# ignacio-rocco/detectorch

Hardware: AMD Instinct MI355X
Metric: images/sec Mask R-CNN R-50-FPN 1333x800 (region-proposal hot path) (higher is better)
Workload: dtype f32

## Files before the change

### detectorch_amd/csrc/roi_align_common.h

```cpp
#pragma once
#include "dtc_common.h"

namespace dtc {

struct RoiAlignParams {
  dtc_feat_level lv[DTC_MAX_LEVELS];
  const float* rois;
  const int32_t* roi_levels;
  const int32_t* roi_order;
  const float* roi_desc;
  void* out;
  int n_levels, channels, roi_cols, n_rois, pooled_h, pooled_w, sampling_ratio, ch_tile;
  int ch_block;
  int cts64;
  int xcd_remap;
  const void* prep = nullptr;
};

constexpr int kXcds = 8;
__device__ __forceinline__ int xcd_work_item(int b, int n, int enabled) {
  if (!enabled || n < 2 * kXcds) return b;
  const int x = b % kXcds, j = b / kXcds;
  const int q = n / kXcds, r = n - q * kXcds;
  return x * q + min(x, r) + j;
// ... 18 lines not shown
  e.l = valid ? l : 0.f;
  e.h = valid ? h : 0.f;
  return e;
}

struct RoiHead {
  int r, lvl, b;
  float sw, sh, rw, rh;
  float bin_h, bin_w;
  int gh, gw;
  float count, inv_count;
};

struct RoiRaw { float4 d0, d1; };

__device__ __forceinline__ RoiRaw load_roi_raw(const RoiAlignParams& p, int ri) {
  RoiRaw w;
  if (p.roi_desc) {
    w.d0 = reinterpret_cast<const float4*>(p.roi_desc)[(size_t)ri * 2];
    w.d1 = reinterpret_cast<const float4*>(p.roi_desc)[(size_t)ri * 2 + 1];
  } else {
    const int r = p.roi_order ? p.roi_order[ri] : ri;
    const int lvl = p.roi_levels ? p.roi_levels[r] : 0;
    const float* roi = p.rois + (size_t)r * p.roi_cols;
    float b = 0.f;
    if (p.roi_cols == 5) { b = roi[0]; roi++; }
    w.d0 = make_float4(b, roi[0], roi[1], roi[2]);
    w.d1 = make_float4(roi[3], (float)lvl, (float)r, 0.f);
  }
  return w;
}

__device__ __forceinline__ RoiHead roi_head_from_raw(const RoiAlignParams& p, const RoiRaw& w) {
  RoiHead h;
  h.b = (int)w.d0.x; h.lvl = (int)w.d1.y; h.r = (int)w.d1.z;
  const float x1 = w.d0.y, y1 = w.d0.z, x2 = w.d0.w, y2 = w.d1.x;
  h.sw = h.sh = 0.f; h.rw = h.rh = 1.f; h.bin_h = h.bin_w = 1.f; h.gh = h.gw = 1; h.count = 1.f; h.inv_count = 1.f;
  if (h.lvl < 0 || h.lvl >= p.n_levels) return h;
  const float s = p.lv[h.lvl].spatial_scale;
  h.sw = x1 * s; h.sh = y1 * s;
  const float ew = x2 * s, eh = y2 * s;
  h.rw = fmaxf(ew - h.sw, 1.f); h.rh = fmaxf(eh - h.sh, 1.f);
  h.bin_h = fdiv(h.rh, (float)p.pooled_h); h.bin_w = fdiv(h.rw, (float)p.pooled_w);
  h.gh = p.sampling_ratio > 0 ? p.sampling_ratio : (int)ceilf(fdiv(h.rh, (float)p.pooled_h));
  h.gw = p.sampling_ratio > 0 ? p.sampling_ratio : (int)ceilf(fdiv(h.rw, (float)p.pooled_w));
  const int gg = h.gh * h.gw;
  h.count = (float)gg;
  h.inv_count = ((gg & (gg - 1)) == 0) ? fdiv(1.f, h.count) : 0.f;
  return h;
}

__device__ __forceinline__ RoiHead load_roi_head(const RoiAlignParams& p, int ri) {
  return roi_head_from_raw(p, load_roi_raw(p, ri));
}

typedef float f32x2 __attribute__((ext_vector_type(2)));
template <typename T> __device__ __forceinline__ f32x2 mul_pair16(uint32_t u, float w);
template <> __device__ __forceinline__ f32x2 mul_pair16<__half>(uint32_t u, float w) {
  f32x2 r;
  asm("v_fma_mix_f32 %0, %2, %3, %4 op_sel:[0,0,0] op_sel_hi:[1,0,0]\n\tv_fma_mix_f32 %1, %2, %3, %4 op_sel:[1,0,0] op_sel_hi:[1,0,0]"
      : "=&v"(r.x), "=&v"(r.y) : "v"(u), "v"(w), "s"(-0.0f));
  return r;
}
template <> __device__ __forceinline__ f32x2 mul_pair16<bf16_t>(uint32_t u, float w) {
  const f32x2 v = {__uint_as_float(u << 16), __uint_as_float(u & 0xffff0000u)};
  return v * w;
}
template <> __device__ __forceinline__ f32x2 mul_pair16<float>(uint32_t, float) { return f32x2{0.f, 0.f}; }

template <typename T> __device__ __forceinline__ void fma_pair16(f32x2& acc, uint32_t u, float w);
template <> __device__ __forceinline__ void fma_pair16<__half>(f32x2& acc, uint32_t u, float w) {
  asm("v_fma_mix_f32 %0, %2, %3, %0 op_sel:[0,0,0] op_sel_hi:[1,0,0]\n\tv_fma_mix_f32 %1, %2, %3, %1 op_sel:[1,0,0] op_sel_hi:[1,0,0]"
      : "+v"(acc.x), "+v"(acc.y) : "v"(u), "v"(w));
}
template <> __device__ __forceinline__ void fma_pair16<bf16_t>(f32x2& acc, uint32_t u, float w) {
  const f32x2 v = {__uint_as_float(u << 16), __uint_as_float(u & 0xffff0000u)};
  const f32x2 w2 = {w, w};
  acc = __builtin_elementwise_fma(v, w2, acc);
}
template <> __device__ __forceinline__ void fma_pair16<float>(f32x2&, uint32_t, float) {}

bool roi_align_tile_supported(const RoiAlignParams& p, int in_dtype, int out_dtype);
int launch_roi_align_tile(const RoiAlignParams& p, int in_dtype, int out_dtype, hipStream_t stream);
bool roi_align_map_supported(const RoiAlignParams& p, int in_dtype, int out_dtype);
int launch_roi_align_map(const RoiAlignParams& p, int in_dtype, int out_dtype, hipStream_t stream);
void roi_align_set_exact(int exact);
int roi_align_get_exact();
size_t roi_align_map_workspace_bytes(int n_rois);
int launch_roi_align_map_ws(const RoiAlignParams& p, int in_dtype, int out_dtype, void* workspace, size_t workspace_bytes, hipStream_t stream);

bool roi_align_nhwc_lds_supported(const RoiAlignParams& p, int in_dtype, int out_dtype);
int launch_roi_align_nhwc_lds(const RoiAlignParams& p, int in_dtype, int out_dtype, hipStream_t stream);

bool roi_align_nhwc16_supported(const RoiAlignParams& p, int in_dtype, int out_dtype);
int launch_roi_align_nhwc16(const RoiAlignParams& p, int in_dtype, int out_dtype, hipStream_t stream);

}
```

### detectorch_amd/csrc/roi_align_tile.hip

```cpp
#include <stdlib.h>

#include <mutex>
#include <type_traits>

#include "roi_align_common.h"

namespace dtc {

constexpr int kTileMaxK = 32;
constexpr int kTileRoiBytes = 48, kTileGroupBytes = 32;
constexpr int kTileHdrBytes = kTileMaxK * (kTileRoiBytes + kTileGroupBytes) + 16;
template <int NT> struct TileShape;
template <> struct TileShape<256> { static constexpr int kUnits = 8, kWaves = 3, kLdsKB = 52, kWaves16 = 4, kLds16KB = 38; };

struct TileRoi {
  int lvl, b, x0, x1, y0, y1, r, valid;
  float sh, sw, bin_h, bin_w;
};
static_assert(sizeof(TileRoi) == kTileRoiBytes, "TileRoi layout");
struct TileGroup { int first, count, kind, x0, x1, y0, y1, pad; };
enum { kGrpPool = 0, kGrpZero = 1, kGrpAbsent = 2, kGrpGather = 3 };

typedef uint32_t u32x4 __attribute__((ext_vector_type(4)));
typedef uint32_t u32x2 __attribute__((ext_vector_type(2)));
typedef float f32x2 __attribute__((ext_vector_type(2)));
typedef float f32x4 __attribute__((ext_vector_type(4)));
__device__ __forceinline__ __amdgpu_buffer_rsrc_t make_srd(const void* base) {
  return __builtin_amdgcn_make_buffer_rsrc(const_cast<void*>(base), 0, 0xffffffff, 0x00020000);
}
template <typename TIn> struct Piece4;
template <> struct Piece4<float> {
  typedef float4 Raw;
  static __device__ __forceinline__ Raw raw(__amdgpu_buffer_rsrc_t r, uint32_t voff, uint32_t soff) { return ld(r, voff, soff); }
  static __device__ __forceinline__ float4 ld(__amdgpu_buffer_rsrc_t r, uint32_t voff, uint32_t soff) {
    const u32x4 v = __builtin_amdgcn_raw_buffer_load_b128(r, voff, soff, 0);
    return make_float4(__uint_as_float(v.x), __uint_as_float(v.y), __uint_as_float(v.z), __uint_as_float(v.w));
  }
};
template <> struct Piece4<__half> {
  typedef u32x2 Raw;
  static __device__ __forceinline__ Raw raw(__amdgpu_buffer_rsrc_t r, uint32_t voff, uint32_t soff) { return __builtin_amdgcn_raw_buffer_load_b64(r, voff, soff, 0); }
  static __device__ __forceinline__ float4 ld(__amdgpu_buffer_rsrc_t r, uint32_t voff, uint32_t soff) {
    const u32x2 v = __builtin_amdgcn_raw_buffer_load_b64(r, voff, soff, 0);
    const uint32_t x = v.x, y = v.y;
    const __half2 a = *reinterpret_cast<const __half2*>(&x), b = *reinterpret_cast<const __half2*>(&y);
    return make_float4(__low2float(a), __high2float(a), __low2float(b), __high2float(b));
  }
};
template <> struct Piece4<bf16_t> {
  typedef u32x2 Raw;
  static __device__ __forceinline__ Raw raw(__amdgpu_buffer_rsrc_t r, uint32_t voff, uint32_t soff) { return __builtin_amdgcn_raw_buffer_load_b64(r, voff, soff, 0); }
  static __device__ __forceinline__ float4 ld(__amdgpu_buffer_rsrc_t r, uint32_t voff, uint32_t soff) {
    const u32x2 v = __builtin_amdgcn_raw_buffer_load_b64(r, voff, soff, 0);
    return bf16x4_to_f32(make_uint2(v.x, v.y));
  }
};

__device__ __forceinline__ int uni(int v) { return __builtin_amdgcn_readfirstlane(v); }

#ifdef DTC_TILE_TRACE
constexpr int kTraceSlots = 16;
__device__ unsigned long long g_tile_trace[kTraceSlots * 16384];
struct TileTrace {
  unsigned long long last, acc[kTraceSlots];
  __device__ __forceinline__ void start() { for (int i = 0; i < kTraceSlots; i++) acc[i] = 0; last = __builtin_readcyclecounter(); }
  __device__ __forceinline__ void mark(int i) { const unsigned long long n = __builtin_readcyclecounter(); acc[i] += n - last; last = n; }
};
#define TT_MARK(i) tt.mark(i)
#else
struct TileTrace {};
#define TT_MARK(i) ((void)0)
#endif

template <typename TIn> struct TileLds { typedef float T; static constexpr int kSlot = 16, kShift = 4; };
template <> struct TileLds<__half> { typedef uint16_t T; static constexpr int kSlot = 8, kShift = 3; };
template <> struct TileLds<bf16_t> { typedef uint16_t T; static constexpr int kSlot = 8, kShift = 3; };

template <typename TIn, int NT> struct TileBounds { static constexpr int kWaves = TileShape<NT>::kWaves; };
template <int NT> struct TileBounds<__half, NT> { static constexpr int kWaves = TileShape<NT>::kWaves16; };
template <int NT> struct TileBounds<bf16_t, NT> { static constexpr int kWaves = TileShape<NT>::kWaves16; };

__device__ __forceinline__ int tile_phys(int px) { return px + (px >> 3); }

struct TileItem {
  int a[2][2][4];
  float yl[2], yh[2], xl[2], xh[2];
  bool on;
};

template <typename TOut> __device__ __forceinline__ void store_quad(TOut* d, float4 v);
template <> __device__ __forceinline__ void store_quad<float>(float* d, float4 v) { store_stream16(d, v); }
template <> __device__ __forceinline__ void store_quad<__half>(__half* d, float4 v) {
  const __half2 a = __floats2half2_rn(v.x, v.y), b = __floats2half2_rn(v.z, v.w);
  store_stream8(d, *reinterpret_cast<const uint32_t*>(&a), *reinterpret_cast<const uint32_t*>(&b));
}
template <> __device__ __forceinline__ void store_quad<bf16_t>(bf16_t* d, float4 v) {
  store_stream8(d, (uint32_t)from_f32<bf16_t>(v.x).bits | ((uint32_t)from_f32<bf16_t>(v.y).bits << 16),
                (uint32_t)from_f32<bf16_t>(v.z).bits | ((uint32_t)from_f32<bf16_t>(v.w).bits << 16));
}

enum { kStageScalar = 0, kStageVec = 1, kStageVecUnaligned = 2 };

struct TileGeom {
  int first, count;
  int y0, x0a, ngx, npos;
  int plane;
  int nq_pass;
  int mode;
};

template <typename TIn, typename TOut, int NT, bool FUSED>
__device__ __forceinline__ void tile_passes(const RoiAlignParams& p, const dtc_feat_level& L, const TIn* fbase, int c0, int nc,
                                            int bins, float* slab, typename TileLds<TIn>::T* win, const TileRoi* troi, const TileGeom& g,
                                            const TileItem& it, int rl, int bin, TileTrace& tt) {
  constexpr int NW = NT / 64;
  constexpr int U = TileShape<NT>::kUnits;
  typedef typename TileLds<TIn>::T TL;
  constexpr bool L16 = sizeof(TL) == 2;
  constexpr int SB = TileLds<TIn>::kSlot;
  const int tid = threadIdx.x, lane = tid & 63, wv = tid >> 6, pl = lane & 15, cl = (lane >> 4) & 3;
  const int npos = g.npos, ngx = g.ngx, plane = g.plane, nq_pass = g.nq_pass;
  const int nchunk = (npos + 15) >> 4;
  const int KC = ceil_div(nchunk, NW);
  const float rinv = 1.0f / (float)ngx;
  const int nq_tot = ceil_div(nc, 4);
  const bool vec = g.mode != kStageScalar;
  uint32_t uoff[U];
  int ulds[U];
  const int nu = KC * nq_pass;
  if (vec) {
    const int sh32 = (int)L.stride_h, sc32 = (int)L.stride_c;
    int q = 0, i = 0;
#pragma unroll
    for (int u = 0; u < U; u++) {
      const bool dup = u >= nu;
      const int pos = min((wv + (dup ? 0 : i) * NW) * 16 + pl, npos - 1);
      const int row = (int)(((float)pos + 0.5f) * rinv);
      const int gx = pos - row * ngx;
      const int qq = dup ? 0 : q;
      int col = g.x0a + 4 * gx, sft = 0;
      if (g.mode == kStageVecUnaligned) { sft = max(0, col + 3 - (L.width - 1)); col -= sft; }
      uoff[u] = ((uint32_t)((g.y0 + row) * sh32 + col + (4 * qq + cl) * sc32) * (uint32_t)sizeof(TIn)) | ((uint32_t)sft << 30);
      ulds[u] = qq * plane * 4 + ((4 * pos + (pos >> 1)) << 2) + cl;
      if (++i == KC) { i = 0; q++; }
    }
  }
  const __amdgpu_buffer_rsrc_t srd = make_srd(fbase);
  const uint32_t pass_bytes = (uint32_t)(L.stride_c * (int64_t)sizeof(TIn));
  typename Piece4<TIn>::Raw v[U];
  auto issue = [&](int cs) {
    const uint32_t soff = (uint32_t)cs * pass_bytes;
    if (g.mode == kStageVec) {
#pragma unroll
      for (int u = 0; u < U; u++) v[u] = Piece4<TIn>::raw(srd, uoff[u], soff);
    } else {
#pragma unroll
      for (int u = 0; u < U; u++) v[u] = Piece4<TIn>::raw(srd, uoff[u] & 0x3fffffffu, soff);
    }
  };
  auto commit_as = [&](auto shifted_tag) {
    constexpr bool SHIFTED = decltype(shifted_tag)::value;
    if constexpr (SHIFTED) asm volatile("" ::: "memory");
#pragma unroll
    for (int u = 0; u < U; u++) {
      if constexpr (L16) {
        uint32_t w0 = v[u].x & 0xffffu, w1 = v[u].x >> 16, w2 = v[u].y & 0xffffu, w3 = v[u].y >> 16;
        if constexpr (SHIFTED) {
          const uint32_t sft = uoff[u] >> 30;
          w0 = sft == 0 ? w0 : sft == 1 ? w1 : sft == 2 ? w2 : w3;
          w1 = sft == 0 ? w1 : sft == 1 ? w2 : w3;
          w2 = sft == 0 ? w2 : w3;
        }
        TL* d = win + ulds[u];
        d[0] = (TL)w0; d[4] = (TL)w1; d[8] = (TL)w2; d[12] = (TL)w3;
      } else {
        float4 w = v[u];
        if constexpr (SHIFTED) {
          const uint32_t sft = uoff[u] >> 30;
          w.x = sft == 0 ? w.x : sft == 1 ? w.y : sft == 2 ? w.z : w.w;
          w.y = sft == 0 ? w.y : sft == 1 ? w.z : w.w;
          w.z = sft == 0 ? w.z : w.w;
        }
        TL* d = win + ulds[u];
        d[0] = w.x; d[4] = w.y; d[8] = w.z; d[12] = w.w;
// ... 122 lines not shown
    TT_MARK(4);
    if (nq_prev) store_slab(cs_prev, nq_prev);
    TT_MARK(5);
    __syncthreads();
    TT_MARK(6);
    if (vec && qs + nq_pass < nq_tot) issue(cs + 4 * nq_pass);
    TT_MARK(7);
    if (it.on) {
      float* so = slab + rl * (4 * nq_cur * bins) + bin;
#pragma unroll 1
      for (int q = 0; q < nq_cur; q++) {
        const char* wq = reinterpret_cast<const char*>(win) + uni(q * plane * SB);
        f32x2 a01 = {0.f, 0.f}, a23 = {0.f, 0.f};
#pragma unroll
        for (int iy = 0; iy < 2; iy++) {
          if constexpr (L16 && FUSED) {
            u32x2 t[2][4];
#pragma unroll
            for (int ix = 0; ix < 2; ix++)
#pragma unroll
              for (int k = 0; k < 4; k++)
                t[ix][k] = *reinterpret_cast<const u32x2*>(__builtin_assume_aligned(wq + it.a[iy][ix][k], 8));
#pragma unroll
            for (int ix = 0; ix < 2; ix++) {
              const float w1 = it.yh[iy] * it.xh[ix], w2 = it.yh[iy] * it.xl[ix];
              const float w3 = it.yl[iy] * it.xh[ix], w4 = it.yl[iy] * it.xl[ix];
              fma_pair16<TIn>(a01, t[ix][0].x, w1); fma_pair16<TIn>(a23, t[ix][0].y, w1);
              fma_pair16<TIn>(a01, t[ix][1].x, w2); fma_pair16<TIn>(a23, t[ix][1].y, w2);
              fma_pair16<TIn>(a01, t[ix][2].x, w3); fma_pair16<TIn>(a23, t[ix][2].y, w3);
              fma_pair16<TIn>(a01, t[ix][3].x, w4); fma_pair16<TIn>(a23, t[ix][3].y, w4);
            }
          } else if constexpr (L16) {
            u32x2 t[2][4];
#pragma unroll
            for (int ix = 0; ix < 2; ix++)
#pragma unroll
              for (int k = 0; k < 4; k++)
                t[ix][k] = *reinterpret_cast<const u32x2*>(__builtin_assume_aligned(wq + it.a[iy][ix][k], 8));
#pragma unroll
            for (int ix = 0; ix < 2; ix++) {
              const float w1 = it.yh[iy] * it.xh[ix], w2 = it.yh[iy] * it.xl[ix];
              const float w3 = it.yl[iy] * it.xh[ix], w4 = it.yl[iy] * it.xl[ix];
              f32x2 s01 = mul_pair16<TIn>(t[ix][0].x, w1) + mul_pair16<TIn>(t[ix][1].x, w2);
              s01 = s01 + mul_pair16<TIn>(t[ix][2].x, w3);
              s01 = s01 + mul_pair16<TIn>(t[ix][3].x, w4);
              f32x2 s23 = mul_pair16<TIn>(t[ix][0].y, w1) + mul_pair16<TIn>(t[ix][1].y, w2);
              s23 = s23 + mul_pair16<TIn>(t[ix][2].y, w3);
              s23 = s23 + mul_pair16<TIn>(t[ix][3].y, w4);
              a01 = a01 + s01; a23 = a23 + s23;
            }
          } else {
            f32x4 t[2][4];
#pragma unroll
            for (int ix = 0; ix < 2; ix++)
#pragma unroll
              for (int k = 0; k < 4; k++)
                t[ix][k] = *reinterpret_cast<const f32x4*>(__builtin_assume_aligned(wq + it.a[iy][ix][k], 16));
#pragma unroll
            for (int ix = 0; ix < 2; ix++) {
              const float w1 = it.yh[iy] * it.xh[ix], w2 = it.yh[iy] * it.xl[ix];
              const float w3 = it.yl[iy] * it.xh[ix], w4 = it.yl[iy] * it.xl[ix];
              a01 += w1 * t[ix][0].lo + w2 * t[ix][1].lo + w3 * t[ix][2].lo + w4 * t[ix][3].lo;
              a23 += w1 * t[ix][0].hi + w2 * t[ix][1].hi + w3 * t[ix][2].hi + w4 * t[ix][3].hi;
            }
          }
          __builtin_amdgcn_sched_barrier(0);
        }
        float* o = so + uni(4 * q * bins);
        const float a0 = a01.x, a1 = a01.y, a2 = a23.x, a3 = a23.y;
        o[0] = a0 * 0.25f; o[bins] = a1 * 0.25f; o[2 * bins] = a2 * 0.25f; o[3 * bins] = a3 * 0.25f;
      }
    }
    TT_MARK(8);
    __syncthreads();
    TT_MARK(9);
    cs_prev = cs; nq_prev = nq_cur;
  }
  if (nq_prev) store_slab(cs_prev, nq_prev);
  TT_MARK(10);
}
#endif


__device__ __forceinline__ int tile_work_item(int b, int n, int reverse) {
  if (n < 2 * kXcds || (reverse & 2)) return (reverse & 1) ? n - 1 - b : b;
  const int x = b % kXcds, j = b / kXcds;
  const int q = n / kXcds, r = n - q * kXcds;
  const int start = x * q + min(x, r), qx = q + (x < r ? 1 : 0);
  return start + ((reverse & 1) ? qx - 1 - j : j);
}

template <typename TIn, typename TOut, int NT, bool FUSED>
__global__ __launch_bounds__(NT, (TileBounds<TIn, NT>::kWaves)) void roi_align_fwd_tile(RoiAlignParams p, int kgroup, int lds_bytes, int nq_cap, int merge_pct, int reverse) {
  extern __shared__ __attribute__((aligned(16))) unsigned char smem[];
  TileRoi* troi = reinterpret_cast<TileRoi*>(smem);
  TileGroup* tgrp = reinterpret_cast<TileGroup*>(smem + kTileMaxK * kTileRoiBytes);
  int* ngp = reinterpret_cast<int*>(smem + kTileMaxK * (kTileRoiBytes + kTileGroupBytes));
  const int slab_bytes = kgroup * p.pooled_h * p.pooled_w * 16 * nq_cap;
  float* slab = reinterpret_cast<float*>(smem + kTileHdrBytes);
  typedef typename TileLds<TIn>::T TL;
  constexpr int SB = TileLds<TIn>::kSlot;
  TL* win = reinterpret_cast<TL*>(smem + kTileHdrBytes + slab_bytes);
  const int win_bytes = lds_bytes - kTileHdrBytes - slab_bytes;
  constexpr int NW = NT / 64;
  constexpr int kMaxPos = TileShape<NT>::kUnits * NW * 16;
  const int tid = threadIdx.x;
  const int nct = ceil_div(p.channels, p.ch_block);
  int wi = tile_work_item(blockIdx.x, gridDim.x, reverse);
  int grp = wi / nct;
  int c0 = (wi - grp * nct) * p.ch_block;
  {
    const int ngrp = (int)gridDim.x / nct;
    if ((reverse & 4) && ngrp % kXcds == 0 && ngrp >= 2 * kXcds) {
      const int x = blockIdx.x % kXcds, j = blockIdx.x / kXcds, ngx = ngrp / kXcds;
      const int cbi = j / ngx, gl = j - cbi * ngx;
      grp = x * ngx + ((reverse & 1) ? ngx - 1 - gl : gl);
      c0 = cbi * p.ch_block;
      wi = grp * nct + cbi;
    }
  }
  const int nc = min(p.ch_block, p.channels - c0);
  const int bins = p.pooled_h * p.pooled_w;
  const int K = kgroup;
  TileTrace tt;
#ifdef DTC_TILE_TRACE
  tt.start();
  const unsigned long long wall0 = __builtin_amdgcn_s_memrealtime();
#endif

  if (tid < 64) {
    TileRoi t;
    t.lvl = -1; t.b = 0; t.x0 = t.x1 = t.y0 = t.y1 = 0; t.r = 0; t.valid = 0; t.sh = t.sw = 0.f; t.bin_h = t.bin_w = 1.f;
    const int ri = grp * K + tid;
    if (tid < K && ri < p.n_rois) {
      const RoiHead hd = load_roi_head(p, ri);
      t.valid = 1; t.r = hd.r; t.b = hd.b; t.sh = hd.sh; t.sw = hd.sw; t.bin_h = hd.bin_h; t.bin_w = hd.bin_w;
      if (hd.lvl >= 0 && hd.lvl < p.n_levels) {
        t.lvl = hd.lvl;
        const int H = p.lv[hd.lvl].height, W = p.lv[hd.lvl].width;
        t.y0 = make_axis(hd.sh, hd.bin_h, 0, 0, 2, H).lo;
        t.y1 = make_axis(hd.sh, hd.bin_h, p.pooled_h - 1, 1, 2, H).hi;
        t.x0 = make_axis(hd.sw, hd.bin_w, 0, 0, 2, W).lo;
        t.x1 = make_axis(hd.sw, hd.bin_w, p.pooled_w - 1, 1, 2, W).hi;
      }
    }
    if (tid < K) {
      troi[tid] = t;
      *reinterpret_cast<uint64_t*>(&troi[tid].x0) = ((uint64_t)(uint32_t)t.r * (uint64_t)p.channels + (uint64_t)c0) * (uint64_t)(p.pooled_h * p.pooled_w);
    }
    auto bc = [](int v, int k) { return __builtin_amdgcn_readlane(v, k); };
    int ng = 0, k = 0;
    while (k < K) {
      const int ks = uni(k);
      const int a_lvl = bc(t.lvl, ks), a_b = bc(t.b, ks), a_valid = bc(t.valid, ks);
      const int a_x0 = bc(t.x0, ks), a_x1 = bc(t.x1, ks), a_y0 = bc(t.y0, ks), a_y1 = bc(t.y1, ks);
      TileGroup g;
      g.first = k; g.count = 1; g.x0 = a_x0; g.x1 = a_x1; g.y0 = a_y0; g.y1 = a_y1; g.pad = 0;
      if (!a_valid) g.kind = kGrpAbsent;
      else if (a_lvl < 0) g.kind = kGrpZero;
      else {
        const int ngx0 = (a_x1 >> 2) - (a_x0 >> 2) + 1, th0 = a_y1 - a_y0 + 1, npos0 = th0 * ngx0;
        if (npos0 > kMaxPos || (4 * npos0 + (npos0 >> 1) + 1) * SB > win_bytes || bins > NT) {
          g.kind = kGrpGather;
        } else {
          g.kind = kGrpPool;
          long long sum_px = (long long)th0 * (a_x1 - a_x0 + 1);
          while (k + g.count < K && (g.count + 1) * bins <= NT) {
            const int js = uni(k + g.count);
            const int n_lvl = bc(t.lvl, js), n_b = bc(t.b, js), n_valid = bc(t.valid, js);
            if (!n_valid || n_lvl != a_lvl || n_b != a_b) break;
            const int n_x0 = bc(t.x0, js), n_x1 = bc(t.x1, js), n_y0 = bc(t.y0, js), n_y1 = bc(t.y1, js);
            const int ux0 = min(g.x0, n_x0), ux1 = max(g.x1, n_x1), uy0 = min(g.y0, n_y0), uy1 = max(g.y1, n_y1);
            const int ungx = (ux1 >> 2) - (ux0 >> 2) + 1, uth = uy1 - uy0 + 1, unpos = uth * ungx;
// ... 104 lines not shown
    unsigned long long* o = g_tile_trace + (size_t)blockIdx.x * kTraceSlots;
    for (int i = 0; i < 11; i++) o[i] = tt.acc[i];
    o[11] = wall0; o[12] = __builtin_amdgcn_s_memrealtime();
    o[13] = (unsigned long long)ngroups; o[14] = (unsigned long long)__builtin_amdgcn_s_getreg((4 << 0) | (0 << 6) | (31 << 11));
    o[15] = (unsigned long long)wi;
  }
#endif
}

#ifdef DTC_TILE_TRACE
}
extern "C" __attribute__((visibility("default"))) int dtc_debug_tile_trace(void* host_dst, size_t bytes) {
  return hipMemcpyFromSymbol(host_dst, HIP_SYMBOL(dtc::g_tile_trace), bytes, 0, hipMemcpyDeviceToHost) == hipSuccess ? 0 : -1;
}
namespace dtc {
#endif

struct TileConfig {
  int nt = 256;
  int lds_kb = 0;
  int lds16_kb = 0;
  int k = 0;
  int ch_block = 0;
  int merge_pct = 250;
  int nq_cap = 0;
  int reverse = 1;
  int cb_major = 1;
};
static const TileConfig& tile_config() {
  static const TileConfig cfg = [] {
    TileConfig c;
    if (const char* e = getenv("DTC_RA_TILE_CBMAJOR")) c.cb_major = atoi(e) != 0;
    if (const char* e = getenv("DTC_RA_TILE_LDS16_KB")) { const int v = atoi(e); if (v >= 36 && v <= 156) c.lds16_kb = v; }
    if (const char* e = getenv("DTC_RA_TILE_CHBLOCK")) { const int v = atoi(e); if (v >= 4 && (v & 3) == 0) c.ch_block = v; }
    return c;
  }();
  return cfg;
}

template <typename TIn, typename TOut, int NT, bool FUSED>
static int launch_tile_nt(RoiAlignParams p, hipStream_t stream) {
  const TileConfig& cfg = tile_config();
  const int bins = p.pooled_h * p.pooled_w;
  int K = cfg.k ? cfg.k : NT / bins;
  K = K < 1 ? 1 : (K > kTileMaxK ? kTileMaxK : K);
  if (K * bins > NT) K = NT / bins;
  if (K < 1) return DTC_EUNSUPPORTED;
  const int lds_b = (sizeof(TIn) == 2 ? (cfg.lds16_kb ? cfg.lds16_kb : TileShape<NT>::kLds16KB) : cfg.lds_kb ? cfg.lds_kb : TileShape<NT>::kLdsKB) * 1024;
  static std::once_flag once;
  static hipError_t attr_rc = hipSuccess;
  std::call_once(once, [] {
    attr_rc = hipFuncSetAttribute(reinterpret_cast<const void*>(roi_align_fwd_tile<TIn, TOut, NT, FUSED>),
                                  hipFuncAttributeMaxDynamicSharedMemorySize, 160 * 1024);
  });
  if (attr_rc != hipSuccess) return DTC_ELAUNCH;
  const int nq_cap = cfg.nq_cap ? cfg.nq_cap : 4;
  if (kTileHdrBytes + K * bins * 16 * nq_cap + 20 * 1024 > lds_b) return DTC_EUNSUPPORTED;
  const int ngrp = ceil_div(p.n_rois, K);
  int cb = cfg.ch_block ? cfg.ch_block : ((long long)ngrp * ceil_div(p.channels, 128) >= 6144 ? 128 : 64);
  while (!cfg.ch_block && cb > 32 && (long long)ngrp * ceil_div(p.channels, cb) < 2048) cb >>= 1;
  p.ch_block = cb;
  const int nct = ceil_div(p.channels, p.ch_block);
  hipLaunchKernelGGL((roi_align_fwd_tile<TIn, TOut, NT, FUSED>), dim3((unsigned)ngrp * nct), dim3(NT), lds_b, stream, p, K, lds_b, nq_cap, cfg.merge_pct, (cfg.reverse ? 1 : 0) | (p.xcd_remap ? 0 : 2) | (cfg.cb_major ? 4 : 0));
  DTC_CHECK_LAUNCH();
  return DTC_OK;
}

template <typename TIn, typename TOut>
static int launch_tile_t(const RoiAlignParams& p, hipStream_t stream) {
  if constexpr (sizeof(TIn) == 2) { if (!roi_align_get_exact()) return launch_tile_nt<TIn, TOut, 256, true>(p, stream); }
  return launch_tile_nt<TIn, TOut, 256, false>(p, stream);
}

bool roi_align_tile_supported(const RoiAlignParams& p, int in_dtype, int out_dtype) {
  if (p.sampling_ratio != 2) return false;
  if (p.pooled_h * p.pooled_w > tile_config().nt) return false;
  const bool f = in_dtype == DTC_F32, h = in_dtype == DTC_F16, b = in_dtype == DTC_BF16;
  return (f && (out_dtype == DTC_F32 || out_dtype == DTC_F16 || out_dtype == DTC_BF16)) ||
         (h && (out_dtype == DTC_F32 || out_dtype == DTC_F16)) || (b && (out_dtype == DTC_F32 || out_dtype == DTC_BF16));
}

int launch_roi_align_tile(const RoiAlignParams& p, int in_dtype, int out_dtype, hipStream_t stream) {
  if (p.n_rois == 0) return DTC_OK;
  if (in_dtype == DTC_F32 && out_dtype == DTC_F32) return launch_tile_t<float, float>(p, stream);
  if (in_dtype == DTC_F16 && out_dtype == DTC_F32) return launch_tile_t<__half, float>(p, stream);
  if (in_dtype == DTC_F16 && out_dtype == DTC_F16) return launch_tile_t<__half, __half>(p, stream);
  if (in_dtype == DTC_F32 && out_dtype == DTC_F16) return launch_tile_t<float, __half>(p, stream);
  if (in_dtype == DTC_BF16 && out_dtype == DTC_F32) return launch_tile_t<bf16_t, float>(p, stream);
  if (in_dtype == DTC_BF16 && out_dtype == DTC_BF16) return launch_tile_t<bf16_t, bf16_t>(p, stream);
  if (in_dtype == DTC_F32 && out_dtype == DTC_BF16) return launch_tile_t<float, bf16_t>(p, stream);
  return DTC_EUNSUPPORTED;
}

}
```

Before: 14370.

## Add dedicated mask-head RoIAlign kernel with per-ROI channel-block tiling

Adds a specialized RoIAlign kernel for large pooled outputs (over 128 bins, e.g. the 14x14 mask head). Each block handles one ROI and one channel block: it stages the ROI's feature window into LDS with buffer loads double-buffered across channel quads, then computes bilinear samples from LDS, with XCD-aware work ordering. The tile launcher dispatches to this path when it is supported. Shared helpers move into a new header. This adds a separate code path whose benefit depends on how many ROIs and which pooled sizes the benchmark actually uses.

```diff
diff --git a/detectorch_amd/csrc/roi_align_common.h b/detectorch_amd/csrc/roi_align_common.h
--- a/detectorch_amd/csrc/roi_align_common.h
+++ b/detectorch_amd/csrc/roi_align_common.h
@@ -124,6 +124,8 @@
 
 bool roi_align_tile_supported(const RoiAlignParams& p, int in_dtype, int out_dtype);
 int launch_roi_align_tile(const RoiAlignParams& p, int in_dtype, int out_dtype, hipStream_t stream);
+bool roi_align_mask_supported(const RoiAlignParams& p, int in_dtype, int out_dtype);
+int launch_roi_align_mask(const RoiAlignParams& p, int in_dtype, int out_dtype, hipStream_t stream);
 bool roi_align_map_supported(const RoiAlignParams& p, int in_dtype, int out_dtype);
 int launch_roi_align_map(const RoiAlignParams& p, int in_dtype, int out_dtype, hipStream_t stream);
 void roi_align_set_exact(int exact);
diff --git a/detectorch_amd/csrc/roi_align_mask.hip b/detectorch_amd/csrc/roi_align_mask.hip
--- /dev/null
+++ b/detectorch_amd/csrc/roi_align_mask.hip
@@ -0,0 +1,330 @@
+#include <stdlib.h>
+
+#include <mutex>
+
+#include "roi_align_stage.h"
+
+namespace dtc {
+
+constexpr int kMaskNT = 256;
+constexpr int kMaskUnits = 8;
+template <typename TIn> struct MaskShape { static constexpr int kWaves = 3, kLdsKB = 52, kQuads = 8; };
+template <> struct MaskShape<__half> { static constexpr int kWaves = 4, kLdsKB = 38, kQuads = 4; };
+template <> struct MaskShape<bf16_t> { static constexpr int kWaves = 4, kLdsKB = 38, kQuads = 4; };
+
+__device__ __forceinline__ void mask_work_item(int b, int n_rows, int nct, int& row, int& cb) {
+  if (n_rows % kXcds == 0 && n_rows >= 2 * kXcds) {
+    const int x = b % kXcds, j = b / kXcds, ngx = n_rows / kXcds;
+    cb = j / ngx;
+    row = x * ngx + (ngx - 1 - (j - cb * ngx));
+  } else {
+    const int wi = tile_work_item(b, n_rows * nct, 1);
+    row = wi / nct;
+    cb = wi - row * nct;
+  }
+}
+
+template <typename TIn, typename TOut>
+__global__ __launch_bounds__(kMaskNT, MaskShape<TIn>::kWaves) void roi_align_fwd_mask(RoiAlignParams p, int lds_bytes, int nq_cap) {
+  extern __shared__ __attribute__((aligned(16))) unsigned char smem[];
+  typedef typename TileLds<TIn>::T TL;
+  constexpr bool L16 = sizeof(TL) == 2;
+  constexpr int SB = TileLds<TIn>::kSlot, SS = TileLds<TIn>::kShift;
+  constexpr int NT = kMaskNT, NW = NT / 64, U = kMaskUnits;
+  const int tid = threadIdx.x, lane = tid & 63, wv = tid >> 6, pl = lane & 15, cl = (lane >> 4) & 3;
+  const int bins = p.pooled_h * p.pooled_w;
+  const int nc = p.ch_block;
+  const int nct = p.channels / nc;
+  int row, cb;
+  mask_work_item(blockIdx.x, p.n_rois, nct, row, cb);
+  const int c0 = cb * nc;
+  const RoiHead hd = load_roi_head(p, row);
+  TOut* out = reinterpret_cast<TOut*>(p.out) + ((size_t)hd.r * p.channels + c0) * bins;
+  if (hd.lvl < 0 || hd.lvl >= p.n_levels) {
+    for (int o = tid; o < nc * bins; o += NT) out[o] = from_f32<TOut>(0.f);
+    return;
+  }
+  const dtc_feat_level L = p.lv[hd.lvl];
+  const TIn* fbase = reinterpret_cast<const TIn*>(L.data) + (int64_t)hd.b * L.stride_n + (int64_t)c0 * L.stride_c;
+  const int y0 = make_axis(hd.sh, hd.bin_h, 0, 0, 2, L.height).lo;
+  const int y1 = make_axis(hd.sh, hd.bin_h, p.pooled_h - 1, 1, 2, L.height).hi;
+  const int x0 = make_axis(hd.sw, hd.bin_w, 0, 0, 2, L.width).lo;
+  const int x1 = make_axis(hd.sw, hd.bin_w, p.pooled_w - 1, 1, 2, L.width).hi;
+  const int x0a = x0 & ~3, ngx = (x1 >> 2) - (x0 >> 2) + 1, tw = 4 * ngx;
+  const int npos = (y1 - y0 + 1) * ngx;
+  const int plane = 4 * npos + (npos >> 1) + 1;
+  const int nchunk = (npos + 15) >> 4, KC = ceil_div(nchunk, NW);
+  const int slab_bytes = bins * 16 * nq_cap;
+  const int img_bytes = lds_bytes - slab_bytes;
+  float* slab = reinterpret_cast<float*>(smem);
+  TL* win = reinterpret_cast<TL*>(smem + slab_bytes);
+
+  if (KC > U || plane * SB > img_bytes) {
+    for (int o = tid; o < nc * bins; o += NT) {
+      const int c = o / bins, bin = o - c * bins;
+      const int ph = bin / p.pooled_w, pw = bin - ph * p.pooled_w;
+      const TIn* d = fbase + (int64_t)c * L.stride_c;
+      float acc = 0.f;
+      for (int iy = 0; iy < 2; iy++) {
+        const AxisEntry y = make_axis(hd.sh, hd.bin_h, ph, iy, 2, L.height);
+        const int64_t ylo = (int64_t)y.lo * L.stride_h, yhi = (int64_t)y.hi * L.stride_h;
+        for (int ix = 0; ix < 2; ix++) {
+          const AxisEntry x = make_axis(hd.sw, hd.bin_w, pw, ix, 2, L.width);
+          const int64_t xlo = (int64_t)x.lo * L.stride_w, xhi = (int64_t)x.hi * L.stride_w;
+          const float w1 = y.h * x.h, w2 = y.h * x.l, w3 = y.l * x.h, w4 = y.l * x.l;
+          acc += w1 * to_f32<TIn>(d[ylo + xlo]) + w2 * to_f32<TIn>(d[ylo + xhi]) + w3 * to_f32<TIn>(d[yhi + xlo]) +
+                 w4 * to_f32<TIn>(d[yhi + xhi]);
+        }
+      }
+      out[o] = from_f32<TOut>(acc * 0.25f);
+    }
+    return;
+  }
+  const bool al16 = ((L.width | L.stride_h | L.stride_c | L.stride_n) & 3) == 0 &&
+                    (reinterpret_cast<uintptr_t>(L.data) & (4 * sizeof(TIn) - 1)) == 0;
+  const int nq_tot = nc >> 2;
+  int nq_pass = max(1, min(min(img_bytes / (plane * SB), U / KC), min(nq_tot, nq_cap)));
+  while (nq_tot % nq_pass) nq_pass--;
+
+  const int nu = KC * nq_pass;
+  const float rinv = 1.0f / (float)ngx;
+  uint32_t uoff[U];
+  int ulds[U];
+  {
+    const int sh32 = (int)L.stride_h, sc32 = (int)L.stride_c;
+    int q = 0, i = 0;
+#pragma unroll
+    for (int u = 0; u < U; u++) {
+      const bool dup = u >= nu;
+      const int pos = min((wv + (dup ? 0 : i) * NW) * 16 + pl, npos - 1);
+      const int r = (int)(((float)pos + 0.5f) * rinv);
+      const int gx = pos - r * ngx;
+      const int qq = dup ? 0 : q;
+      int col = x0a + 4 * gx, sft = 0;
+      if (!al16) { sft = max(0, col + 3 - (L.width - 1)); col -= sft; }
+      uoff[u] = ((uint32_t)((y0 + r) * sh32 + col + (4 * qq + cl) * sc32) * (uint32_t)sizeof(TIn)) | ((uint32_t)sft << 30);
+      ulds[u] = qq * plane * 4 + ((4 * pos + (pos >> 1)) << 2) + cl;
+      if (++i == KC) { i = 0; q++; }
+    }
+  }
+  const __amdgpu_buffer_rsrc_t srd = make_srd(fbase);
+  const uint32_t pass_bytes = (uint32_t)(L.stride_c * (int64_t)sizeof(TIn));
+  typename Piece4<TIn>::Raw v[U];
+  auto issue = [&](int cs) {
+    const uint32_t soff = (uint32_t)cs * pass_bytes;
+    if (al16) {
+#pragma unroll
+      for (int u = 0; u < U; u++) v[u] = Piece4<TIn>::raw(srd, uoff[u], soff);
+    } else {
+#pragma unroll
+      for (int u = 0; u < U; u++) v[u] = Piece4<TIn>::raw(srd, uoff[u] & 0x3fffffffu, soff);
+    }
+  };
+  auto commit_as = [&](auto shifted_tag) {
+    constexpr bool SHIFTED = decltype(shifted_tag)::value;
+    if constexpr (SHIFTED) asm volatile("" ::: "memory");
+#pragma unroll
+    for (int u = 0; u < U; u++) {
+      if constexpr (L16) {
+        uint32_t w0 = v[u].x & 0xffffu, w1 = v[u].x >> 16, w2 = v[u].y & 0xffffu, w3 = v[u].y >> 16;
+        if constexpr (SHIFTED) {
+          const uint32_t sft = uoff[u] >> 30;
+          w0 = sft == 0 ? w0 : sft == 1 ? w1 : sft == 2 ? w2 : w3;
+          w1 = sft == 0 ? w1 : sft == 1 ? w2 : w3;
+          w2 = sft == 0 ? w2 : w3;
+        }
+        TL* d = win + ulds[u];
+        d[0] = (TL)w0; d[4] = (TL)w1; d[8] = (TL)w2; d[12] = (TL)w3;
+      } else {
+        float4 w = v[u];
+        if constexpr (SHIFTED) {
+          const uint32_t sft = uoff[u] >> 30;
+          w.x = sft == 0 ? w.x : sft == 1 ? w.y : sft == 2 ? w.z : w.w;
+          w.y = sft == 0 ? w.y : sft == 1 ? w.z : w.w;
+          w.z = sft == 0 ? w.z : w.w;
+        }
+        TL* d = win + ulds[u];
+        d[0] = w.x; d[4] = w.y; d[8] = w.z; d[12] = w.w;
+      }
+    }
+  };
+  auto commit = [&]() {
+    if (!al16) commit_as(std::true_type{}); else commit_as(std::false_type{});
+  };
+  auto store_slab = [&](int cs, int nq) {
+    const int n4 = nq * bins;
+    TOut* o = out + cs * bins;
+    for (int idx = tid; idx < n4; idx += NT) store_quad<TOut>(o + 4 * idx, reinterpret_cast<const float4*>(slab)[idx]);
+  };
+
+  issue(0);
+
+  const bool on = tid < bins;
+  const int bin = on ? tid : 0;
+  const int ph = bin / p.pooled_w, pw = bin - ph * p.pooled_w;
+  int a[2][2][4];
+  float yl[2], yh[2], xl[2], xh[2];
+  {
+    int ylo[2], yhi[2], xlo[2], xhi[2];
+#pragma unroll
+    for (int i = 0; i < 2; i++) {
+      const AxisEntry ey = make_axis(hd.sh, hd.bin_h, ph, i, 2, L.height);
+      const AxisEntry ex = make_axis(hd.sw, hd.bin_w, pw, i, 2, L.width);
+      yl[i] = ey.l; yh[i] = ey.h; xl[i] = ex.l; xh[i] = ex.h;
+      ylo[i] = (ey.lo - y0) * tw; yhi[i] = (ey.hi - y0) * tw;
+      xlo[i] = ex.lo - x0a; xhi[i] = ex.hi - x0a;
+    }
+#pragma unroll
+    for (int iy = 0; iy < 2; iy++)
+#pragma unroll
+      for (int ix = 0; ix < 2; ix++) {
+        int t0 = tile_phys(ylo[iy] + xlo[ix]) << SS, t1 = tile_phys(ylo[iy] + xhi[ix]) << SS;
+        int t2 = tile_phys(yhi[iy] + xlo[ix]) << SS, t3 = tile_phys(yhi[iy] + xhi[ix]) << SS;
+        asm volatile("" : "+v"(t0), "+v"(t1), "+v"(t2), "+v"(t3));
+        a[iy][ix][0] = t0; a[iy][ix][1] = t1; a[iy][ix][2] = t2; a[iy][ix][3] = t3;
+      }
+  }
+
+  int cs_prev = 0, nq_prev = 0;
+#pragma unroll 1
+  for (int qs = 0; qs < nq_tot; qs += nq_pass) {
+    const int cs = 4 * qs;
+    commit();
+    if (nq_prev) store_slab(cs_prev, nq_prev);
+    __syncthreads();
+    if (qs + nq_pass < nq_tot) issue(cs + 4 * nq_pass);
+    if (on) {
+      float* so = slab + bin;
+#pragma unroll 1
+      for (int q = 0; q < nq_pass; q++) {
+        const char* wq = reinterpret_cast<const char*>(win) + uni(q * plane * SB);
+        f32x2 a01 = {0.f, 0.f}, a23 = {0.f, 0.f};
+#pragma unroll
+        for (int iy = 0; iy < 2; iy++) {
+          if constexpr (L16) {
+            u32x2 t[2][4];
+#pragma unroll
+            for (int ix = 0; ix < 2; ix++)
+#pragma unroll
+              for (int k = 0; k < 4; k++) t[ix][k] = *reinterpret_cast<const u32x2*>(__builtin_assume_aligned(wq + a[iy][ix][k], 8));
+#pragma unroll
+            for (int ix = 0; ix < 2; ix++) {
+              const float w1 = yh[iy] * xh[ix], w2 = yh[iy] * xl[ix];
+              const float w3 = yl[iy] * xh[ix], w4 = yl[iy] * xl[ix];
+              f32x2 s01 = mul_pair16<TIn>(t[ix][0].x, w1) + mul_pair16<TIn>(t[ix][1].x, w2);
+              s01 = s01 + mul_pair16<TIn>(t[ix][2].x, w3);
+              s01 = s01 + mul_pair16<TIn>(t[ix][3].x, w4);
+              f32x2 s23 = mul_pair16<TIn>(t[ix][0].y, w1) + mul_pair16<TIn>(t[ix][1].y, w2);
+              s23 = s23 + mul_pair16<TIn>(t[ix][2].y, w3);
+              s23 = s23 + mul_pair16<TIn>(t[ix][3].y, w4);
+              a01 = a01 + s01; a23 = a23 + s23;
+            }
+          } else {
+            f32x4 t[2][4];
+#pragma unroll
+            for (int ix = 0; ix < 2; ix++)
+#pragma unroll
+              for (int k = 0; k < 4; k++) t[ix][k] = *reinterpret_cast<const f32x4*>(__builtin_assume_aligned(wq + a[iy][ix][k], 16));
+#pragma unroll
+            for (int ix = 0; ix < 2; ix++) {
+              const float w1 = yh[iy] * xh[ix], w2 = yh[iy] * xl[ix];
+              const float w3 = yl[iy] * xh[ix], w4 = yl[iy] * xl[ix];
+              a01 += w1 * t[ix][0].lo + w2 * t[ix][1].lo + w3 * t[ix][2].lo + w4 * t[ix][3].lo;
+              a23 += w1 * t[ix][0].hi + w2 * t[ix][1].hi + w3 * t[ix][2].hi + w4 * t[ix][3].hi;
+            }
+          }
+          __builtin_amdgcn_sched_barrier(0);
+        }
+        float* o = so + uni(4 * q * bins);
+        o[0] = a01.x * 0.25f; o[bins] = a01.y * 0.25f; o[2 * bins] = a23.x * 0.25f; o[3 * bins] = a23.y * 0.25f;
+      }
+    }
+    __syncthreads();
+    cs_prev = cs; nq_prev = nq_pass;
+  }
+  store_slab(cs_prev, nq_prev);
+}
+
+struct MaskConfig {
+  int enabled = 1;
+  int ch_block = 0;
+  int lds_kb = 0;
+  int quads = 0;
+};
+static const MaskConfig& mask_config() {
+  static const MaskConfig cfg = [] {
+    MaskConfig c;
+    if (const char* e = getenv("DTC_RA_MASK")) c.enabled = atoi(e) != 0;
+    if (const char* e = getenv("DTC_RA_MASK_CHBLOCK")) { const int v = atoi(e); if (v == 32 || v == 64 || v == 128) c.ch_block = v; }
+    if (const char* e = getenv("DTC_RA_MASK_LDS_KB")) { const int v = atoi(e); if (v >= 32 && v <= 156) c.lds_kb = v; }
+    if (const char* e = getenv("DTC_RA_MASK_QUADS")) { const int v = atoi(e); if (v >= 1 && v <= 8) c.quads = v; }
+    return c;
+  }();
+  return cfg;
+}
+
+static int mask_ch_block(const RoiAlignParams& p) {
+  const MaskConfig& cfg = mask_config();
+  if (cfg.ch_block) return p.channels % cfg.ch_block == 0 ? cfg.ch_block : 0;
+  int cb = 64;
+  while (cb > 32 && (long long)p.n_rois * (p.channels / cb) < 2048) cb >>= 1;
+  return p.channels % cb == 0 ? cb : (p.channels % 32 == 0 ? 32 : 0);
+}
+
+bool roi_align_mask_supported(const RoiAlignParams& p, int in_dtype, int out_dtype) {
+  const int bins = p.pooled_h * p.pooled_w;
+  if (!mask_config().enabled || !p.roi_desc || p.sampling_ratio != 2 || bins <= 128 || bins > kMaskNT) return false;
+  const bool f = in_dtype == DTC_F32, h = in_dtype == DTC_F16, b = in_dtype == DTC_BF16;
+  if (!((f && (out_dtype == DTC_F32 || out_dtype == DTC_F16 || out_dtype == DTC_BF16)) ||
+        (h && (out_dtype == DTC_F32 || out_dtype == DTC_F16)) || (b && (out_dtype == DTC_F32 || out_dtype == DTC_BF16))))
+    return false;
+  if (!f && !roi_align_get_exact()) return false;
+  if (mask_ch_block(p) == 0) return false;
+  const int esz = f ? 4 : 2;
+  for (int i = 0; i < p.n_levels; i++) {
+    const dtc_feat_level& L = p.lv[i];
+    const bool lin = L.stride_w == 1 && L.stride_h > 0 && L.stride_c > 0 && L.stride_n >= 0 &&
+                     L.stride_h * L.height + L.stride_c * 4 * kMaskUnits < (1ll << 26);
+    const bool al16 = ((L.width | L.stride_h | L.stride_c | L.stride_n) & 3) == 0 &&
+                      (reinterpret_cast<uintptr_t>(L.data) & (4 * esz - 1)) == 0;
+    const bool al4 = L.width >= 4 && (((L.width | L.stride_h | L.stride_c | L.stride_n) * esz) & 3) == 0 &&
+                     (reinterpret_cast<uintptr_t>(L.data) & 3) == 0;
+    if (!lin || !(al16 || al4)) return false;
+  }
+  return true;
+}
+
+template <typename TIn, typename TOut>
+static int launch_mask_t(RoiAlignParams p, hipStream_t stream) {
+  const MaskConfig& cfg = mask_config();
+  const int lds_b = (cfg.lds_kb ? cfg.lds_kb : MaskShape<TIn>::kLdsKB) * 1024;
+  const int nq_cap = cfg.quads ? cfg.quads : MaskShape<TIn>::kQuads;
+  if (p.pooled_h * p.pooled_w * 16 * nq_cap + 4 * 1024 > lds_b) return DTC_EUNSUPPORTED;
+  static std::once_flag once;
+  static hipError_t attr_rc = hipSuccess;
+  std::call_once(once, [] {
+    attr_rc = hipFuncSetAttribute(reinterpret_cast<const void*>(roi_align_fwd_mask<TIn, TOut>), hipFuncAttributeMaxDynamicSharedMemorySize,
+                                  160 * 1024);
+  });
+  if (attr_rc != hipSuccess) return DTC_ELAUNCH;
+  p.ch_block = mask_ch_block(p);
+  const long long grid = (long long)p.n_rois * (p.channels / p.ch_block);
+  if (grid > 0x7fffffff) return DTC_EUNSUPPORTED;
+  hipLaunchKernelGGL((roi_align_fwd_mask<TIn, TOut>), dim3((unsigned)grid), dim3(kMaskNT), lds_b, stream, p, lds_b, nq_cap);
+  DTC_CHECK_LAUNCH();
+  return DTC_OK;
+}
+
+int launch_roi_align_mask(const RoiAlignParams& p, int in_dtype, int out_dtype, hipStream_t stream) {
+  if (p.n_rois == 0) return DTC_OK;
+  if (in_dtype == DTC_F32 && out_dtype == DTC_F32) return launch_mask_t<float, float>(p, stream);
+  if (in_dtype == DTC_F16 && out_dtype == DTC_F32) return launch_mask_t<__half, float>(p, stream);
+  if (in_dtype == DTC_F16 && out_dtype == DTC_F16) return launch_mask_t<__half, __half>(p, stream);
+  if (in_dtype == DTC_F32 && out_dtype == DTC_F16) return launch_mask_t<float, __half>(p, stream);
+  if (in_dtype == DTC_BF16 && out_dtype == DTC_F32) return launch_mask_t<bf16_t, float>(p, stream);
+  if (in_dtype == DTC_BF16 && out_dtype == DTC_BF16) return launch_mask_t<bf16_t, bf16_t>(p, stream);
+  if (in_dtype == DTC_F32 && out_dtype == DTC_BF16) return launch_mask_t<float, bf16_t>(p, stream);
+  return DTC_EUNSUPPORTED;
+}
+
+}
diff --git a/detectorch_amd/csrc/roi_align_stage.h b/detectorch_amd/csrc/roi_align_stage.h
--- /dev/null
+++ b/detectorch_amd/csrc/roi_align_stage.h
@@ -0,0 +1,70 @@
+#pragma once
+#include "roi_align_common.h"
+
+namespace dtc {
+
+typedef uint32_t u32x4 __attribute__((ext_vector_type(4)));
+typedef uint32_t u32x2 __attribute__((ext_vector_type(2)));
+typedef float f32x2 __attribute__((ext_vector_type(2)));
+typedef float f32x4 __attribute__((ext_vector_type(4)));
+__device__ __forceinline__ __amdgpu_buffer_rsrc_t make_srd(const void* base) {
+  return __builtin_amdgcn_make_buffer_rsrc(const_cast<void*>(base), 0, 0xffffffff, 0x00020000);
+}
+template <typename TIn> struct Piece4;
+template <> struct Piece4<float> {
+  typedef float4 Raw;
+  static __device__ __forceinline__ Raw raw(__amdgpu_buffer_rsrc_t r, uint32_t voff, uint32_t soff) { return ld(r, voff, soff); }
+  static __device__ __forceinline__ float4 ld(__amdgpu_buffer_rsrc_t r, uint32_t voff, uint32_t soff) {
+    const u32x4 v = __builtin_amdgcn_raw_buffer_load_b128(r, voff, soff, 0);
+    return make_float4(__uint_as_float(v.x), __uint_as_float(v.y), __uint_as_float(v.z), __uint_as_float(v.w));
+  }
+};
+template <> struct Piece4<__half> {
+  typedef u32x2 Raw;
+  static __device__ __forceinline__ Raw raw(__amdgpu_buffer_rsrc_t r, uint32_t voff, uint32_t soff) { return __builtin_amdgcn_raw_buffer_load_b64(r, voff, soff, 0); }
+  static __device__ __forceinline__ float4 ld(__amdgpu_buffer_rsrc_t r, uint32_t voff, uint32_t soff) {
+    const u32x2 v = __builtin_amdgcn_raw_buffer_load_b64(r, voff, soff, 0);
+    const uint32_t x = v.x, y = v.y;
+    const __half2 a = *reinterpret_cast<const __half2*>(&x), b = *reinterpret_cast<const __half2*>(&y);
+    return make_float4(__low2float(a), __high2float(a), __low2float(b), __high2float(b));
+  }
+};
+template <> struct Piece4<bf16_t> {
+  typedef u32x2 Raw;
+  static __device__ __forceinline__ Raw raw(__amdgpu_buffer_rsrc_t r, uint32_t voff, uint32_t soff) { return __builtin_amdgcn_raw_buffer_load_b64(r, voff, soff, 0); }
+  static __device__ __forceinline__ float4 ld(__amdgpu_buffer_rsrc_t r, uint32_t voff, uint32_t soff) {
+    const u32x2 v = __builtin_amdgcn_raw_buffer_load_b64(r, voff, soff, 0);
+    return bf16x4_to_f32(make_uint2(v.x, v.y));
+  }
+};
+
+__device__ __forceinline__ int uni(int v) { return __builtin_amdgcn_readfirstlane(v); }
+
+template <typename TIn> struct TileLds { typedef float T; static constexpr int kSlot = 16, kShift = 4; };
+template <> struct TileLds<__half> { typedef uint16_t T; static constexpr int kSlot = 8, kShift = 3; };
+template <> struct TileLds<bf16_t> { typedef uint16_t T; static constexpr int kSlot = 8, kShift = 3; };
+
+__device__ __forceinline__ int tile_phys(int px) { return px + (px >> 3); }
+
+template <typename TOut> __device__ __forceinline__ void store_quad(TOut* d, float4 v);
+template <> __device__ __forceinline__ void store_quad<float>(float* d, float4 v) { store_stream16(d, v); }
+template <> __device__ __forceinline__ void store_quad<__half>(__half* d, float4 v) {
+  const __half2 a = __floats2half2_rn(v.x, v.y), b = __floats2half2_rn(v.z, v.w);
+  store_stream8(d, *reinterpret_cast<const uint32_t*>(&a), *reinterpret_cast<const uint32_t*>(&b));
+}
+template <> __device__ __forceinline__ void store_quad<bf16_t>(bf16_t* d, float4 v) {
+  store_stream8(d, (uint32_t)from_f32<bf16_t>(v.x).bits | ((uint32_t)from_f32<bf16_t>(v.y).bits << 16),
+                (uint32_t)from_f32<bf16_t>(v.z).bits | ((uint32_t)from_f32<bf16_t>(v.w).bits << 16));
+}
+
+enum { kStageScalar = 0, kStageVec = 1, kStageVecUnaligned = 2 };
+
+__device__ __forceinline__ int tile_work_item(int b, int n, int reverse) {
+  if (n < 2 * kXcds || (reverse & 2)) return (reverse & 1) ? n - 1 - b : b;
+  const int x = b % kXcds, j = b / kXcds;
+  const int q = n / kXcds, r = n - q * kXcds;
+  const int start = x * q + min(x, r), qx = q + (x < r ? 1 : 0);
+  return start + ((reverse & 1) ? qx - 1 - j : j);
+}
+
+}
diff --git a/detectorch_amd/csrc/roi_align_tile.hip b/detectorch_amd/csrc/roi_align_tile.hip
--- a/detectorch_amd/csrc/roi_align_tile.hip
+++ b/detectorch_amd/csrc/roi_align_tile.hip
@@ -3,7 +3,7 @@
 #include <mutex>
 #include <type_traits>
 
-#include "roi_align_common.h"
+#include "roi_align_stage.h"
 
 namespace dtc {
 
@@ -21,42 +21,6 @@
 struct TileGroup { int first, count, kind, x0, x1, y0, y1, pad; };
 enum { kGrpPool = 0, kGrpZero = 1, kGrpAbsent = 2, kGrpGather = 3 };
 
-typedef uint32_t u32x4 __attribute__((ext_vector_type(4)));
-typedef uint32_t u32x2 __attribute__((ext_vector_type(2)));
-typedef float f32x2 __attribute__((ext_vector_type(2)));
-typedef float f32x4 __attribute__((ext_vector_type(4)));
-__device__ __forceinline__ __amdgpu_buffer_rsrc_t make_srd(const void* base) {
-  return __builtin_amdgcn_make_buffer_rsrc(const_cast<void*>(base), 0, 0xffffffff, 0x00020000);
-}
-template <typename TIn> struct Piece4;
-template <> struct Piece4<float> {
-  typedef float4 Raw;
-  static __device__ __forceinline__ Raw raw(__amdgpu_buffer_rsrc_t r, uint32_t voff, uint32_t soff) { return ld(r, voff, soff); }
-  static __device__ __forceinline__ float4 ld(__amdgpu_buffer_rsrc_t r, uint32_t voff, uint32_t soff) {
-    const u32x4 v = __builtin_amdgcn_raw_buffer_load_b128(r, voff, soff, 0);
-    return make_float4(__uint_as_float(v.x), __uint_as_float(v.y), __uint_as_float(v.z), __uint_as_float(v.w));
-  }
-};
-template <> struct Piece4<__half> {
-  typedef u32x2 Raw;
-  static __device__ __forceinline__ Raw raw(__amdgpu_buffer_rsrc_t r, uint32_t voff, uint32_t soff) { return __builtin_amdgcn_raw_buffer_load_b64(r, voff, soff, 0); }
-  static __device__ __forceinline__ float4 ld(__amdgpu_buffer_rsrc_t r, uint32_t voff, uint32_t soff) {
-    const u32x2 v = __builtin_amdgcn_raw_buffer_load_b64(r, voff, soff, 0);
-    const uint32_t x = v.x, y = v.y;
-    const __half2 a = *reinterpret_cast<const __half2*>(&x), b = *reinterpret_cast<const __half2*>(&y);
-    return make_float4(__low2float(a), __high2float(a), __low2float(b), __high2float(b));
-  }
-};
-template <> struct Piece4<bf16_t> {
-  typedef u32x2 Raw;
-  static __device__ __forceinline__ Raw raw(__amdgpu_buffer_rsrc_t r, uint32_t voff, uint32_t soff) { return __builtin_amdgcn_raw_buffer_load_b64(r, voff, soff, 0); }
-  static __device__ __forceinline__ float4 ld(__amdgpu_buffer_rsrc_t r, uint32_t voff, uint32_t soff) {
-    const u32x2 v = __builtin_amdgcn_raw_buffer_load_b64(r, voff, soff, 0);
-    return bf16x4_to_f32(make_uint2(v.x, v.y));
-  }
-};
-
-__device__ __forceinline__ int uni(int v) { return __builtin_amdgcn_readfirstlane(v); }
 
 #ifdef DTC_TILE_TRACE
 constexpr int kTraceSlots = 16;
@@ -72,15 +36,11 @@
 #define TT_MARK(i) ((void)0)
 #endif
 
-template <typename TIn> struct TileLds { typedef float T; static constexpr int kSlot = 16, kShift = 4; };
-template <> struct TileLds<__half> { typedef uint16_t T; static constexpr int kSlot = 8, kShift = 3; };
-template <> struct TileLds<bf16_t> { typedef uint16_t T; static constexpr int kSlot = 8, kShift = 3; };
 
 template <typename TIn, int NT> struct TileBounds { static constexpr int kWaves = TileShape<NT>::kWaves; };
 template <int NT> struct TileBounds<__half, NT> { static constexpr int kWaves = TileShape<NT>::kWaves16; };
 template <int NT> struct TileBounds<bf16_t, NT> { static constexpr int kWaves = TileShape<NT>::kWaves16; };
 
-__device__ __forceinline__ int tile_phys(int px) { return px + (px >> 3); }
 
 struct TileItem {
   int a[2][2][4];
@@ -88,18 +48,6 @@
   bool on;
 };
 
-template <typename TOut> __device__ __forceinline__ void store_quad(TOut* d, float4 v);
-template <> __device__ __forceinline__ void store_quad<float>(float* d, float4 v) { store_stream16(d, v); }
-template <> __device__ __forceinline__ void store_quad<__half>(__half* d, float4 v) {
-  const __half2 a = __floats2half2_rn(v.x, v.y), b = __floats2half2_rn(v.z, v.w);
-  store_stream8(d, *reinterpret_cast<const uint32_t*>(&a), *reinterpret_cast<const uint32_t*>(&b));
-}
-template <> __device__ __forceinline__ void store_quad<bf16_t>(bf16_t* d, float4 v) {
-  store_stream8(d, (uint32_t)from_f32<bf16_t>(v.x).bits | ((uint32_t)from_f32<bf16_t>(v.y).bits << 16),
-                (uint32_t)from_f32<bf16_t>(v.z).bits | ((uint32_t)from_f32<bf16_t>(v.w).bits << 16));
-}
-
-enum { kStageScalar = 0, kStageVec = 1, kStageVecUnaligned = 2 };
 
 struct TileGeom {
   int first, count;
@@ -388,13 +336,6 @@
 #endif
 
 
-__device__ __forceinline__ int tile_work_item(int b, int n, int reverse) {
-  if (n < 2 * kXcds || (reverse & 2)) return (reverse & 1) ? n - 1 - b : b;
-  const int x = b % kXcds, j = b / kXcds;
-  const int q = n / kXcds, r = n - q * kXcds;
-  const int start = x * q + min(x, r), qx = q + (x < r ? 1 : 0);
-  return start + ((reverse & 1) ? qx - 1 - j : j);
-}
 
 template <typename TIn, typename TOut, int NT, bool FUSED>
 __global__ __launch_bounds__(NT, (TileBounds<TIn, NT>::kWaves)) void roi_align_fwd_tile(RoiAlignParams p, int kgroup, int lds_bytes, int nq_cap, int merge_pct, int reverse) {
@@ -665,6 +606,7 @@
 
 int launch_roi_align_tile(const RoiAlignParams& p, int in_dtype, int out_dtype, hipStream_t stream) {
   if (p.n_rois == 0) return DTC_OK;
+  if (roi_align_mask_supported(p, in_dtype, out_dtype)) return launch_roi_align_mask(p, in_dtype, out_dtype, stream);
   if (in_dtype == DTC_F32 && out_dtype == DTC_F32) return launch_tile_t<float, float>(p, stream);
   if (in_dtype == DTC_F16 && out_dtype == DTC_F32) return launch_tile_t<__half, float>(p, stream);
   if (in_dtype == DTC_F16 && out_dtype == DTC_F16) return launch_tile_t<__half, __half>(p, stream);
```

Measured after the change: 14590, median of 6. 1.02x the previous value.
